# xianlopez/optical_flow

Measured on AMD Instinct MI355X. Metric: image-pairs/sec training, 384x512 batch=8 per GPU, higher is better.
Workload: dtype fp32

## Files before the change

### optical_flow_amd/csrc/conv_f32.hip

```cpp
#include "common.h"
#include "conv_dev.h"
#include "conv_narrow.h"

#include <algorithm>

namespace oflow {

template <int BM, int BN, int WAVES_M, int WAVES_N, int MODE>
__global__ __launch_bounds__(256, 2) void conv_gemm_f32(GemmArgs a) {
  constexpr int WM = BM / WAVES_M, WN = BN / WAVES_N;
  constexpr int TM = WM / 32, TN = WN / 32;
  static_assert(WAVES_M * WAVES_N == 4, "4 waves");
  static_assert(TM >= 1 && TN >= 1 && WM % 32 == 0 && WN % 32 == 0, "tile");
  constexpr bool A_KCONTIG = (MODE != MODE_WGRAD);
  constexpr int SA = BM + 4;
  constexpr int SB = BN + 4;
  constexpr int A_SLOTS = BM * BK / 4 / 256;
  constexpr int B_QUADS = BK * BN / 4;
  constexpr int B_SLOTS = (B_QUADS + 255) / 256;
  static_assert(A_SLOTS >= 1, "BM >= 64");

  static_assert(2 * BK * (SA + SB) >= 4 * 1024, "epilogue images fit LDS");
  __shared__ float smem[2 * BK * (SA + SB)];
  float (*As)[BK * SA] = reinterpret_cast<float (*)[BK * SA]>(smem);
// ... 602 lines not shown
      return;
    }
#pragma unroll
    for (int i = 0; i < TM; ++i)
#pragma unroll
      for (int j = 0; j < TN; ++j) {
        float4 vv[4];
        int64_t rows[4];
        unsigned ok = 0;
        int ncol = 0;
        transpose32(E, acc[i][j], lane, [&](int row, int c4, float4 v) {
          const int q = row >> 3;
          const int m = m0 + wm0 + 32 * i + row, n = n0 + wn0 + 32 * j + 4 * c4;
          if (a.splits > 1) {
            if (m < M && n < a.N)
              *reinterpret_cast<float4*>(&S[(int64_t)(row_base + m) * a.slab_ld + n]) = v;
            return;
          }
          rows[q] = out_row(a, G, min(m, M - 1));
          ok |= (m < M && n < a.N ? 1u : 0u) << q;
          vv[q] = v;
          ncol = n;
        });
        if (a.splits == 1) epilogue_rows4c<MODE, 4>(a, 0, rows, ok, ncol, min(ncol, a.N - 4), vv);
      }
    return;
  }
  if (a.splits > 1) {
    float* S = a.slab + (int64_t)split * a.split_stride;
    const int row_base = G.tiles_begin * BM;
#pragma unroll
    for (int j = 0; j < TN; ++j) {
      const int n = n0 + wn0 + 32 * j + lrow;
      if (n >= a.N) continue;
#pragma unroll
      for (int i = 0; i < TM; ++i)
#pragma unroll
        for (int r = 0; r < 16; ++r) {
          const int m = m0 + wm0 + 32 * i + (r & 3) + 8 * (r >> 2) + 4 * lk;
          if (m < M) S[(int64_t)(row_base + m) * a.slab_ld + n] = acc[i][j][r];
        }
    }
    return;
  }
#pragma unroll
  for (int j = 0; j < TN; ++j) {
    const int n = n0 + wn0 + 32 * j + lrow;
    if (n >= a.N) continue;
    float bias, scale, shift;
    column_params<MODE>(a, n, bias, scale, shift);
#pragma unroll
    for (int i = 0; i < TM; ++i) {
#pragma unroll
      for (int r0 = 0; r0 < 16; r0 += EP_GATHER<MODE>) {
        EpAux aux[EP_GATHER<MODE>];
#pragma unroll
        for (int r = r0; r < r0 + EP_GATHER<MODE>; ++r) {
          const int m = m0 + wm0 + 32 * i + (r & 3) + 8 * (r >> 2) + 4 * lk;
          aux[r - r0] = m < M ? epilogue_aux<MODE>(a, out_row(a, G, m), n) : EpAux{0.f, 0.f};
        }
#pragma unroll
        for (int r = r0; r < r0 + EP_GATHER<MODE>; ++r) {
          const int m = m0 + wm0 + 32 * i + (r & 3) + 8 * (r >> 2) + 4 * lk;
          if (m >= M) continue;
          epilogue_store<MODE>(a, out_row(a, G, m), n, acc[i][j][r], bias, scale, shift,
                               aux[r - r0]);
        }
      }
    }
  }
}

constexpr int TT_H = 8, TT_W = 16;
#ifndef OF_X3_TH0
#define OF_X3_TH0 8
#endif
constexpr int X3_TH0 = OF_X3_TH0;
#ifndef X3_ABL
#define X3_ABL 0
#endif
#ifndef X3_BDMA
#define X3_BDMA 1
#endif
#ifndef X3_EPB
#define X3_EPB 1
#endif

#ifndef X3_HREC
#define X3_HREC 1
#endif


template <int BN, int WAVES_M, int WAVES_N, int MODE, int TH = OF_TF_H, int PF = 1>
__global__ __launch_bounds__(64 * WAVES_M * WAVES_N, 256 / (32 * WAVES_M * WAVES_N)) void conv_tile_bf16(GemmArgs a) {
  constexpr bool g_tile16_pf_dev = PF != 0;
  constexpr int NT = 64 * WAVES_M * WAVES_N;
  constexpr int BM = TH * TF_W, KS = 3;
  constexpr int HH = TH + KS - 1, HW = TF_W + KS - 1, HP = HH * HW;
  constexpr int WM = BM / WAVES_M, WN = BN / WAVES_N;
  constexpr int TM = WM / 32, TN = WN / 32;
  static_assert((NT == 256 || NT == 512) && TM >= 1 && TN >= 1, "tile");
  constexpr int HQ = HP * 8, HS = (HQ + NT - 1) / NT;
  constexpr int BOCT = KS * BN * 4, BSL = (BOCT + NT - 1) / NT;
  static_assert((HP + 2 * KS * BN) * SROW16 * 16 >= (NT / 64) * 4096, "epilogue images fit LDS");
  __shared__ uint4 smem[(HP + 2 * KS * BN) * SROW16];
  uint4* Ah = smem;
  uint4 (*Bs)[KS * BN * SROW16] = reinterpret_cast<uint4 (*)[KS * BN * SROW16]>(smem + HP * SROW16);

  const int tid = threadIdx.x;
  const int lane = tid & 63;
  const int wave = __builtin_amdgcn_readfirstlane(tid >> 6);
  const int wgid = xcd_remap(blockIdx.x, gridDim.x);
  const int split = wgid / a.tiles_total;
  const int tile = wgid - split * a.tiles_total;
  const int tile_n = tile % a.n_tiles;
  const int tile_m = tile / a.n_tiles;
  const int n0 = tile_n * BN;
  const int OH = MODE == MODE_FWD ? a.ho : a.h, OW = MODE == MODE_FWD ? a.wo : a.w;
  const int SH = MODE == MODE_FWD ? a.h : a.ho, SW = MODE == MODE_FWD ? a.w : a.wo;
  const int tiles_x = (OW + TF_W - 1) / TF_W, tiles_y = (OH + TH - 1) / TH;
  const int b = tile_m / (tiles_x * tiles_y);
  const int trem = tile_m - b * tiles_x * tiles_y;
  const int oy0 = (trem / tiles_x) * TH, ox0 = (trem % tiles_x) * TF_W;
  const int hy0 = MODE == MODE_FWD ? oy0 - a.pt : oy0 + a.pt - (KS - 1);
  const int hx0 = MODE == MODE_FWD ? ox0 - a.pl : ox0 + a.pl - (KS - 1);
  const int c_begin = split * a.k_per_split;
  const int c_end = min(a.K, c_begin + a.k_per_split);
  const int steps = c_end > c_begin ? (c_end - c_begin) * KS : 0;

  const rsrc_t ra_src = make_rsrc(a.A, a.a_bytes);
  const rsrc_t rb_src = make_rsrc(a.B, a.b_bytes);

  int h_off[HS];
  unsigned h_ok = 0;
  const int hcq = tid & 7;
#pragma unroll
  for (int j = 0; j < HS; ++j) {
    const int q = tid + NT * j;
    const int hp = q >> 3;
    const int sy = hy0 + hp / HW, sx = hx0 + hp % HW;
    const bool ok = q < HQ && (unsigned)sy < (unsigned)SH && (unsigned)sx < (unsigned)SW;
    h_off[j] = ok ? (((b * SH + sy) * SW + sx) * a.lda + 4 * hcq) * 4 : 0;
    h_ok |= (ok ? 1u : 0u) << j;
  }
  float4 hv[HS];
  auto load_halo = [&](int c) {
    const bool cok = 32 * c + 4 * hcq < a.kc;
#pragma unroll
    for (int j = 0; j < HS; ++j)
      hv[j] = bload4(ra_src, cok && ((h_ok >> j) & 1) ? (uint32_t)(h_off[j] + 128 * c) : kOOB);
  };
  auto store_halo = [&]() {
#pragma unroll
    for (int j = 0; j < HS; ++j) {
      const int q = tid + NT * j;
      if (q < HQ) {
        bf16x8 t;
        const float4 v = hv[j];
        typedef __bf16 bf16x4 __attribute__((ext_vector_type(4)));
        bf16x4 u;
        u[0] = (__bf16)v.x;
        u[1] = (__bf16)v.y;
        u[2] = (__bf16)v.z;
        u[3] = (__bf16)v.w;
        (void)t;
        *reinterpret_cast<bf16x4*>(reinterpret_cast<char*>(Ah) + (q >> 3) * (SROW16 * 16) +
// ... 175 lines not shown
    __syncthreads();
    if (tid < BN / 4 && n0 + 4 * tid < a.N) {
      float4 sb = red[tid], sg = red[WAVES_M * (BN / 4) + tid];
      for (int w2 = 1; w2 < WAVES_M; ++w2) {
        add4(sb, red[w2 * (BN / 4) + tid]);
        add4(sg, red[(WAVES_M + w2) * (BN / 4) + tid]);
      }
      float* prow = a.bnp + (int64_t)tile_m * 2 * a.N + n0 + 4 * tid;
      *reinterpret_cast<float4*>(prow) = sb;
      *reinterpret_cast<float4*>(prow + a.N) = sg;
    }
    return;
  }
  if (a.vec_ep) {
    float* E = reinterpret_cast<float*>(smem) + wave * 1024;
#pragma unroll
    for (int i = 0; i < TM; ++i)
#pragma unroll
      for (int j = 0; j < TN; ++j) {
        float4 vv[4];
        int64_t rows[4];
        unsigned ok = 0;
        int ncol = 0;
        transpose32(E, acc[i][j], lane, [&](int row, int c4, float4 v) {
          const int q = row >> 3;
          const int mt = wm0 + 32 * i + row, n = n0 + wn0 + 32 * j + 4 * c4;
          const int oy = oy0 + mt / TF_W, ox = ox0 + mt % TF_W;
          rows[q] = img + (int64_t)min(oy, OH - 1) * OW + min(ox, OW - 1);
          ok |= (oy < OH && ox < OW && n < a.N ? 1u : 0u) << q;
          vv[q] = v;
          ncol = n;
        });
        epilogue_rows4c<MODE, 4>(a, split, rows, ok, ncol, min(ncol, a.N - 4), vv);
      }
    return;
  }
#pragma unroll
  for (int j = 0; j < TN; ++j) {
    const int n = n0 + wn0 + 32 * j + lrow;
    if (n >= a.N) continue;
    float bias = 0.f, scale = 1.f, shift = 0.f;
    if (a.splits == 1) column_params<MODE>(a, n, bias, scale, shift);
#pragma unroll
    for (int i = 0; i < TM; ++i) {
      EpAux aux[16];
#pragma unroll
      for (int rr = 0; rr < 16; ++rr) {
        const int m = wm0 + 32 * i + (rr & 3) + 8 * (rr >> 2) + 4 * lk;
        const int oy = oy0 + m / TF_W, ox = ox0 + m % TF_W;
        aux[rr] = a.splits == 1 && oy < OH && ox < OW
                      ? epilogue_aux<MODE>(a, img + (int64_t)oy * OW + ox, n) : EpAux{0.f, 0.f};
      }
#pragma unroll
      for (int rr = 0; rr < 16; ++rr) {
        const int m = wm0 + 32 * i + (rr & 3) + 8 * (rr >> 2) + 4 * lk;
        const int oy = oy0 + m / TF_W, ox = ox0 + m % TF_W;
        if (oy >= OH || ox >= OW) continue;
        const int64_t row = img + (int64_t)oy * OW + ox;
        if (a.splits > 1)
          a.slab[(int64_t)split * a.split_stride + row * a.slab_ld + n] = acc[i][j][rr];
        else
          epilogue_store<MODE>(a, row, n, acc[i][j][rr], bias, scale, shift, aux[rr]);
      }
    }
  }
}

__device__ __forceinline__ void split3x4(const float4& v, uint2& h, uint2& m, uint2& l) {
  const float x[4] = {v.x, v.y, v.z, v.w};
  uint32_t hb[4], mb[4], lb[4];
#pragma unroll
  for (int e = 0; e < 4; ++e) {
    hb[e] = __float_as_uint(x[e]) & 0xffff0000u;
    const float r = x[e] - __uint_as_float(hb[e]);
    mb[e] = __float_as_uint(r) & 0xffff0000u;
    lb[e] = __float_as_uint(r - __uint_as_float(mb[e]));
  }
  auto hi2 = [](uint32_t e0, uint32_t e1) { return __builtin_amdgcn_perm(e1, e0, 0x07060302u); };
  h = make_uint2(hi2(hb[0], hb[1]), hi2(hb[2], hb[3]));
  m = make_uint2(hi2(mb[0], mb[1]), hi2(mb[2], mb[3]));
  l = make_uint2(hi2(lb[0], lb[1]), hi2(lb[2], lb[3]));
}

template <int BN, int WAVES_M, int WAVES_N, int MODE, int TH, int NB, int NP>
__device__ __forceinline__ void tile_x3_body(const GemmArgs& a) {
  constexpr int BM = TH * TF_W, KS = 3;
  static_assert(NP == 1 || NP == 3, "planes");
  constexpr int HH = TH + KS - 1, HW = TF_W + KS - 1, HP = HH * HW;
  constexpr int WM = BM / WAVES_M, WN = BN / WAVES_N;
  constexpr int SM = WM / 16, SN = WN / 16;
  constexpr int NT = 64 * WAVES_M * WAVES_N;
  static_assert(NT % 64 == 0 && NT <= 1024 && WM % 16 == 0 && WN % 16 == 0 && SM >= 1 && SN >= 1,
                "tile");
  constexpr int HQ = HP * 8, HS = (HQ + NT - 1) / NT;
  constexpr int BOCT = NP * BN * 4, BSL = (BOCT + NT - 1) / NT;
  constexpr int AH_U4 = NP * HP * 4, BS_U4 = NB * NP * BN * 4;
  constexpr int EP1_U4 = (NT / 64) * WM * 16 * 4 / 16;
  constexpr int SM_U4 = AH_U4 + BS_U4 > EP1_U4 ? AH_U4 + BS_U4 : EP1_U4;
  constexpr int LDS_B = SM_U4 * 16;
  constexpr int EJ = (NT / 64) * WM * 16 * SN * 4 <= LDS_B ? SN
                     : (NT / 64) * WM * 8 * SN * 4 <= LDS_B ? SN / 2 : 1;
  constexpr int EPW = 16 * EJ;
  static_assert(SN % EJ == 0 && (NT / 64) * WM * EPW * 4 <= LDS_B, "epilogue image fits LDS");
  __shared__ uint4 smem[SM_U4];
  uint4* Ah = smem;
  uint4* Bs = smem + AH_U4;

  const int tid = threadIdx.x;
  const int lane = tid & 63;
  const int wave = __builtin_amdgcn_readfirstlane(tid >> 6);
  const int wgid = xcd_remap(blockIdx.x, gridDim.x);
  const int split = wgid / a.tiles_total;
  const int tile = wgid - split * a.tiles_total;
  const int tile_n = tile % a.n_tiles;
  const int tile_m = tile / a.n_tiles;
  const int n0 = tile_n * BN;
  const int OH = MODE == MODE_FWD ? a.ho : a.h, OW = MODE == MODE_FWD ? a.wo : a.w;
  const int SH = MODE == MODE_FWD ? a.h : a.ho, SW = MODE == MODE_FWD ? a.w : a.wo;
  const int tiles_x = (OW + TF_W - 1) / TF_W, tiles_y = (OH + TH - 1) / TH;
  const int b = tile_m / (tiles_x * tiles_y);
  const int trem = tile_m - b * tiles_x * tiles_y;
  const int oy0 = (trem / tiles_x) * TH, ox0 = (trem % tiles_x) * TF_W;
  const int hy0 = MODE == MODE_FWD ? oy0 - a.pt : oy0 + a.pt - (KS - 1);
  const int hx0 = MODE == MODE_FWD ? ox0 - a.pl : ox0 + a.pl - (KS - 1);
  const int c_begin = split * a.k_per_split;
  const int c_end = min(a.K, c_begin + a.k_per_split);

  const rsrc_t ra_src = make_rsrc(a.A, a.a_bytes);
  const rsrc_t rb_src = make_rsrc(a.B, a.b_bytes);

  float4 hv[HS];
  constexpr bool HREC = X3_HREC && NT == 256 && NP == 3;
  int h_off[HREC ? 1 : HS];
  unsigned h_ok = 0;
  const int hcq = tid & 7;
  auto halo_slot = [&](int t, int j, bool& ok) {
    const int q = t + NT * j;
    const int hp = q >> 3;
    const int sy = hy0 + hp / HW, sx = hx0 + hp % HW;
    ok = q < HQ && (unsigned)sy < (unsigned)SH && (unsigned)sx < (unsigned)SW;
    return ok ? (((b * SH + sy) * SW + sx) * a.lda + 4 * (t & 7)) * 4 : 0;
  };
  if constexpr (!HREC) {
#pragma unroll
    for (int j = 0; j < HS; ++j) {
      bool ok;
      h_off[j] = halo_slot(tid, j, ok);
      h_ok |= (ok ? 1u : 0u) << j;
    }
  }
  auto load_halo = [&](int c) {
    const bool cok = 32 * c + 4 * hcq < a.kc;
    if constexpr (HREC) {
      int t = tid;
      asm volatile("" : "+v"(t));
#pragma unroll
      for (int j = 0; j < HS; ++j) {
        bool ok;
        const int off = halo_slot(t, j, ok);
        hv[j] = bload4(ra_src, cok && ok ? (uint32_t)(off + 128 * c) : kOOB);
      }
    } else {
#pragma unroll
      for (int jj = 0; jj < HS; ++jj)
        hv[jj] = bload4(ra_src, cok && ((h_ok >> jj) & 1) ? (uint32_t)(h_off[jj] + 128 * c) : kOOB);
    }
  };
  auto store_halo = [&]() {
#pragma unroll
    for (int j = 0; j < HS; ++j) {
      const int q = tid + NT * j;
      if (q < HQ) {
        const int hp = q >> 3;
        const int off = hp * 64 + ((((q & 7) >> 1) ^ x3_sw(hp)) << 4) + 8 * (q & 1);
        char* base = reinterpret_cast<char*>(Ah);
        if constexpr (NP == 1) {
          *reinterpret_cast<uint2*>(base + off) = pack_bf16x4(hv[j]);
        } else {
          uint2 h, m, l;
          split3x4(hv[j], h, m, l);
          *reinterpret_cast<uint2*>(base + off) = h;
          *reinterpret_cast<uint2*>(base + HP * 64 + off) = m;
          *reinterpret_cast<uint2*>(base + 2 * HP * 64 + off) = l;
        }
      }
    }
  };
  uint32_t b_off[BSL];
  int b_lds[BSL];
#pragma unroll
  for (int j = 0; j < BSL; ++j) {
    const int o = tid + NT * j;
    const int p = o / (BN * 4), rem = o - p * (BN * 4);
    const int row = rem >> 2, oct = rem & 3;
    const int n = n0 + row;
    const bool ok = o < BOCT && n < a.nb;
    b_off[j] = ok ? (uint32_t)(((int64_t)p * a.b_plane + (int64_t)n * a.ldb + 8 * oct) * 2) : kOOB;
    b_lds[j] = o < BOCT ? (p * BN + row) * 4 + (oct ^ x3_sw(row)) : -1;
  }
  uint4 rb[BSL];
  auto load_b = [&](int c, int t) {
    const int so = (t * a.kc + 32 * c) * 2;
#pragma unroll
    for (int j = 0; j < BSL; ++j)
      rb[j] = __builtin_bit_cast(uint4, __builtin_amdgcn_raw_buffer_load_b128(rb_src, b_off[j], so, 0));
  };
  auto store_b = [&](int buf) {
#pragma unroll
    for (int j = 0; j < BSL; ++j)
      if (BOCT % NT == 0 || b_lds[j] >= 0) Bs[buf * NP * BN * 4 + b_lds[j]] = rb[j];
  };
  constexpr bool BDMA = X3_BDMA && NB == 2;
  constexpr int NW = NT / 64, BDI = NP * BN / 16, BDW = (BDI + NW - 1) / NW;
  uint32_t bd_off[BDW];
  int bd_lds[BDW];
#pragma unroll
  for (int k = 0; k < BDW; ++k) {
    const int g = wave + NW * k;
    const int p = g / (BN / 16), rbk = g % (BN / 16);
    const int n = rbk * 16 + (lane >> 2), o = (lane & 3) ^ x3_sw(lane >> 2);
    bd_off[k] = g < BDI && n0 + n < a.nb
                    ? (uint32_t)(((int64_t)p * a.b_plane + (int64_t)(n0 + n) * a.ldb + 8 * o) * 2)
                    : kOOB;
    bd_lds[k] = g < BDI ? (p * BN + rbk * 16) * 4 : -1;
  }
  auto dma_b = [&](int c, int t, int buf) {
    const int so = (t * a.kc + 32 * c) * 2;
#pragma unroll
    for (int k = 0; k < BDW; ++k)
      if (BDI % NW == 0 || bd_lds[k] >= 0)
        dma16_to_lds(rb_src, Bs + buf * NP * BN * 4 + bd_lds[k], bd_off[k], so);
  };

  f32x4 acc4[SM][SN];
#pragma unroll
  for (int i = 0; i < SM; ++i)
#pragma unroll
    for (int j = 0; j < SN; ++j)
#pragma unroll
      for (int r = 0; r < 4; ++r) acc4[i][j][r] = 0.f;
  const int wm0 = (wave / WAVES_N) * WM;
  const int wn0 = (wave % WAVES_N) * WN;
  const int l16 = lane & 15, lq = lane >> 4;
  int a_hp16[SM];
#pragma unroll
  for (int i = 0; i < SM; ++i) {
    const int m = wm0 + 16 * i + l16;
    const int ty = m / TF_W, tx = m % TF_W;
    a_hp16[i] = MODE == MODE_FWD ? ty * HW + tx : (ty + KS - 1) * HW + tx + KS - 1;
  }
  const int b_frag = (wn0 + l16) * 4 + (lq ^ x3_sw(l16));

  if (c_end > c_begin) {
    load_halo(c_begin);
    if constexpr (BDMA) dma_b(c_begin, 0, 0);
    else load_b(c_begin, 0);
    store_halo();
    if constexpr (!BDMA) store_b(0);
  }
  if constexpr (BDMA) asm volatile("s_waitcnt vmcnt(0)" ::: "memory");
  __syncthreads();
  for (int c = c_begin; c < c_end; ++c) {
    const int cc = c - c_begin;
    const bool more_c = c + 1 < c_end;
    if (more_c && !(X3_ABL & 4)) load_halo(c + 1);
#pragma unroll
    for (int t = 0; t < KS * KS; ++t) {
      const int buf = NB == 2 ? (cc + t) & 1 : 0;
      const bool more = t + 1 < KS * KS || more_c;
      if (more && !(X3_ABL & 2)) {
        if constexpr (BDMA) dma_b(t + 1 < KS * KS ? c : c + 1, t + 1 < KS * KS ? t + 1 : 0, buf ^ 1);
        else load_b(t + 1 < KS * KS ? c : c + 1, t + 1 < KS * KS ? t + 1 : 0);
      }
      __builtin_amdgcn_sched_barrier(0);
      const int r = t / KS, s = t % KS;
      const int dh = MODE == MODE_FWD ? r * HW + s : -(r * HW + s);
      bf16x8 av[NP][SM], bv[NP][SN];
#pragma unroll
      for (int i = 0; i < SM; ++i) {
        const int px = a_hp16[i] + dh;
        const int ai = px * 4 + (lq ^ x3_sw(px));
#pragma unroll
        for (int p = 0; p < NP; ++p) av[p][i] = __builtin_bit_cast(bf16x8, Ah[p * HP * 4 + ai]);
      }
#pragma unroll
      for (int p = 0; p < NP; ++p)
#pragma unroll
        for (int j = 0; j < SN; ++j)
          bv[p][j] = __builtin_bit_cast(bf16x8, Bs[(buf * NP + p) * BN * 4 + 64 * j + b_frag]);
#pragma unroll
      for (int i = 0; i < SM; ++i)
#pragma unroll
        for (int j = 0; j < SN; ++j) {
          f32x4 x = acc4[i][j];
          if constexpr (NP == 1) {
            acc4[i][j] = __builtin_amdgcn_mfma_f32_16x16x32_bf16(av[0][i], bv[0][j], x, 0, 0, 0);
            continue;
          } else {
          if (X3_ABL & 8) {
            asm volatile("" ::"v"(av[1][i]), "v"(av[2][i]), "v"(bv[1][j]), "v"(bv[2][j]));
            acc4[i][j] = __builtin_amdgcn_mfma_f32_16x16x32_bf16(av[0][i], bv[0][j], x, 0, 0, 0);
            continue;
          }
          x = __builtin_amdgcn_mfma_f32_16x16x32_bf16(av[2][i], bv[0][j], x, 0, 0, 0);
          x = __builtin_amdgcn_mfma_f32_16x16x32_bf16(av[0][i], bv[2][j], x, 0, 0, 0);
          x = __builtin_amdgcn_mfma_f32_16x16x32_bf16(av[1][i], bv[1][j], x, 0, 0, 0);
          x = __builtin_amdgcn_mfma_f32_16x16x32_bf16(av[1][i], bv[0][j], x, 0, 0, 0);
          x = __builtin_amdgcn_mfma_f32_16x16x32_bf16(av[0][i], bv[1][j], x, 0, 0, 0);
          acc4[i][j] = __builtin_amdgcn_mfma_f32_16x16x32_bf16(av[0][i], bv[0][j], x, 0, 0, 0);
          }
        }
      __builtin_amdgcn_sched_barrier(0);
      if (!(X3_ABL & 1) && (NB == 1 ? more : (t + 1 == KS * KS && more_c))) __syncthreads();
      if (more) {
        if (!(X3_ABL & 2) && !BDMA) store_b(NB == 2 ? buf ^ 1 : 0);
        if (t + 1 == KS * KS && more_c && !(X3_ABL & 4)) store_halo();
      }
      if constexpr (BDMA) asm volatile("s_waitcnt vmcnt(0)" ::: "memory");
      if (!(X3_ABL & 1)) __syncthreads();
    }
  }

  const int64_t img = (int64_t)b * OH * OW;
  if constexpr (X3_ABL & 16) {
    float v = 0.f;
#pragma unroll
    for (int i = 0; i < SM; ++i)
#pragma unroll
      for (int j = 0; j < SN; ++j) v += acc4[i][j][0] + acc4[i][j][1] + acc4[i][j][2] + acc4[i][j][3];
    a.C[(img + (int64_t)oy0 * OW + ox0) * a.ldc + (n0 + wn0 + (lane & 31)) % a.N] = v;
    return;
  }
  if constexpr (MODE == MODE_FWD && SM % 2 == 0 &&
                (NT / 64) * (WM / 2) * (WN * 4 + 32) <= LDS_B &&
                ((WM / 2) * (WN / 4)) % 64 == 0) {
    if (a.direct16) {
      direct_fwd_f32<SM, SN, WM, WN, TF_W>(
          a, acc4, reinterpret_cast<char*>(smem) + wave * (WM / 2) * (WN * 4 + 32), lane, wm0,
          wn0, n0, oy0, ox0, OH, OW, img);
      return;
    }
  }
  if constexpr (MODE == MODE_DGRAD && NT >= 512 && SM % 2 == 0 &&
                (NT / 64) * (WM / 2) * (WN * 4 + 32) <= LDS_B &&
                ((WM / 2) * (WN / 4)) % 64 == 0) {
    if (a.direct16) {
      direct_dgrad_f32<SM, SN, WM, WN, TF_W>(
          a, acc4, reinterpret_cast<char*>(smem) + wave * (WM / 2) * (WN * 4 + 32), lane, wm0,
          wn0, n0, oy0, ox0, OH, OW, img);
      return;
    }
  }
  if (a.vec_ep) {
    float* E = reinterpret_cast<float*>(smem) + wave * WM * EPW;
    constexpr int LPR = 4 * EJ, RPI = 64 / LPR;
    const int c4 = lane % LPR, rr = lane / LPR;
    constexpr int NPASS = SN / EJ;
    const bool bnp = MODE == MODE_DGRAD && a.bnp != nullptr;
    float4 bsb[NPASS], bsg[NPASS];
#pragma unroll
    for (int p = 0; p < NPASS; ++p) bsb[p] = bsg[p] = make_float4(0.f, 0.f, 0.f, 0.f);
#pragma unroll
    for (int jp = 0; jp < SN; jp += EJ) {
#pragma unroll
      for (int i = 0; i < SM; ++i)
#pragma unroll
        for (int j = 0; j < EJ; ++j)
#pragma unroll
          for (int r = 0; r < 4; ++r)
            E[(16 * i + 4 * lq + r) * EPW + 16 * j + l16] = acc4[i][jp + j][r];
      __builtin_amdgcn_fence(__ATOMIC_RELEASE, "wavefront");
      __builtin_amdgcn_wave_barrier();
      __builtin_amdgcn_fence(__ATOMIC_ACQUIRE, "wavefront");
      const int n = n0 + wn0 + 16 * jp + 4 * c4;
      if constexpr (X3_EPB > 1 && (WM / RPI) % X3_EPB == 0) {
#pragma unroll
        for (int q0 = 0; q0 < WM / RPI; q0 += X3_EPB) {
          float4 v[X3_EPB];
          int64_t row[X3_EPB];
          unsigned ok = 0;
#pragma unroll
          for (int g = 0; g < X3_EPB; ++g) {
            const int m = (q0 + g) * RPI + rr;
            v[g] = *reinterpret_cast<const float4*>(&E[m * EPW + 4 * c4]);
            const int mt = wm0 + m;
            const int oy = oy0 + mt / TF_W, ox = ox0 + mt % TF_W;
            row[g] = img + (int64_t)min(oy, OH - 1) * OW + min(ox, OW - 1);
            ok |= (oy < OH && ox < OW && n < a.N ? 1u : 0u) << g;
          }
          epilogue_rows4c<MODE, X3_EPB>(a, split, row, ok, n, min(n, a.N - 4), v);
        }
      } else if (MODE == MODE_DGRAD && bnp) {
        float4 bt = make_float4(0.f, 0.f, 0.f, 0.f), ig = bt;
        if (n < a.N) {
          bt = *reinterpret_cast<const float4*>(&a.bnp_b[n]);
          const float4 gm = *reinterpret_cast<const float4*>(&a.bnp_g[n]);
          ig = make_float4(1.f / gm.x, 1.f / gm.y, 1.f / gm.z, 1.f / gm.w);
        }
#pragma unroll
        for (int q = 0; q < WM / RPI; ++q) {
          const int m = q * RPI + rr;
          const float4 v = *reinterpret_cast<const float4*>(&E[m * EPW + 4 * c4]);
// ... 3012 lines not shown
  if (st || MODE == MODE_WGRAD || a.splits == 1) return st;
  return launch_splitk_epilogue<MODE>(a, s);
}

template <int MODE>
int launch_gemm_bf16(const GemmArgs& a, hipStream_t s, double flops) {
  const int bn = pick_bn(a.N);
  dim3 grid(a.tiles_total * a.splits), block(256);
  const int cfg = bn == 128 ? 0 : bn == 96 ? 1 : bn == 64 ? 2 : 3;
  if (timing_on()) timing_begin(s);
  if (cfg == 0) hipLaunchKernelGGL((conv_gemm_bf16<128, 128, 2, 2, MODE>), grid, block, 0, s, a);
  else if (cfg == 1) hipLaunchKernelGGL((conv_gemm_bf16<128, 96, 4, 1, MODE>), grid, block, 0, s, a);
  else if (cfg == 2) hipLaunchKernelGGL((conv_gemm_bf16<256, 64, 4, 1, MODE>), grid, block, 0, s, a);
  else hipLaunchKernelGGL((conv_gemm_bf16<256, 32, 4, 1, MODE>), grid, block, 0, s, a);
  if (timing_on()) timing_end(s, 64 + MODE * 8 + cfg, flops);
  int st = check_launch("conv_gemm_bf16");
  if (st || a.splits == 1) return st;
  return launch_splitk_epilogue<MODE>(a, s);
}

bool tile_ok(const of_conv_desc* d) { return d->kh == 3 && d->kw == 3 && d->stride == 1; }

bool x3_tall(int n, int oh, int ow, int N) {
  const int bn = pick_bn(N);
  return (bn == 128 || bn == 96) && (int64_t)n * cdiv(oh, X3_TH0) * cdiv(ow, TF_W) >= 4 * device_cus();
}

constexpr int X3_NB1_MIN = 384;
bool x3_nb1_candidate(const GemmArgs& a, bool tall) {
  return !tall && a.bn_tile == 0 && pick_bn(a.N) == 128 && a.tiles_total >= X3_NB1_MIN;
}
bool x3_nb1(const GemmArgs& a) {
  return a.bm != X3_TH0 * TF_W && a.splits == 1 && x3_nb1_candidate(a, false);
}

static int g_tile_b16 = 0;
bool ws_ok(const of_conv_desc* d, int mode) {
  const int N = mode == MODE_FWD ? d->cout : d->cin_p;
  return (g_tile_b16 == 2 || (g_tile_b16 == 3 && mode == MODE_FWD)) && pick_bn(N) >= 96;
}

static int g_x3t_ep = 5;
static int g_x3g_ep = 5;
static int g_x3_small_bn = 1200;
static int g_x3_bn64 = 0;
static int g_abl_noact = 0;
GemmArgs tile_args(const of_conv_desc* d, const Geo& g, int mode, bool x3 = false,
                   bool b16 = false, bool ws = false) {
  GemmArgs a = base_args(d);
  const bool fwd = mode == MODE_FWD;
  a.kc = fwd ? g.cin_p : g.cout_p;
  a.N = fwd ? d->cout : g.cin_p;
  a.nb = fwd ? d->cout : g.nd;
  a.ldb = fwd ? g.kf16 : (int)g.kd16;
  const int OH = fwd ? d->ho : d->h, OW = fwd ? d->wo : d->w;
  if (x3 && !b16 && !ws && g_x3_small_bn > 0 && pick_bn(a.N) == 128 &&
      (int64_t)d->n * cdiv(OH, TF_H) * cdiv(OW, TF_W) * cdiv(a.N, 128) < g_x3_small_bn)
    a.bn_tile = 64;
  const bool tall64 = x3 && !b16 && !ws && !a.bn_tile && g_x3_bn64 == 1 && pick_bn(a.N) == 64 &&
                      (int64_t)d->n * cdiv(OH, X3_TH0) * cdiv(OW, TF_W) >= 4 * device_cus();
  const bool tall = tall64 ? true : a.bn_tile ? false : ws ? true
                  : x3 || b16 ? x3_tall(d->n, OH, OW, a.N)
                             : (fwd || g_tall16_dgrad) && pick_bn(a.N) == 128 &&
                                   x3_tall(d->n, OH, OW, a.N);
  const int th = tall ? X3_TH0 : TF_H;
  const int m_tiles = d->n * (int)cdiv(OH, th) * (int)cdiv(OW, TF_W);
  a.bm = th * TF_W;
  a.ngroups = 1;
  Group& G = a.grp[0];
  G = Group{};
  G.M = d->n * OH * OW;
  G.m_tiles = m_tiles;
  G.ns = 3;
  G.ntaps = 9;
  a.M = G.M;
  a.n_tiles = (int)cdiv(a.N, a.bn_tile ? a.bn_tile : pick_bn(a.N));
  a.tiles_total = m_tiles * a.n_tiles;
  a.K = (int)cdiv(a.kc, 32);
  G.K = a.K;
  a.splits = 1;
  a.k_per_split = a.K;
  if (x3 || b16 || ws) {
    const bool bn64 = x3 && !b16 && !ws && (a.bn_tile ? a.bn_tile : pick_bn(a.N)) == 64;
    const int slots = !ws && ((b16 && !tall) || x3_nb1_candidate(a, tall) || a.bn_tile == 64 ||
                              (g_x3_bn64 && bn64))
                          ? 2 * device_cus() : device_cus();
    int best = 1;
    double best_cost = 1e30;
    for (int sp = 1; sp <= std::min(8, a.K); ++sp) {
      const int per = (int)cdiv(a.K, sp);
      if (cdiv(a.K, per) != sp) continue;
      const int64_t w = (int64_t)a.tiles_total * sp;
      const double cost = (double)cdiv(w, slots) * (per + 1.0) +
                          (sp > 1 ? 0.1 * g_x3t_ep * sp * a.tiles_total / (double)slots : 0.0);
      if (cost < best_cost - 1e-9) {
        best_cost = cost;
        best = sp;
      }
    }
    a.k_per_split = (int)cdiv(a.K, best);
    a.splits = (int)cdiv(a.K, a.k_per_split);
  } else if (a.tiles_total < 2 * device_cus()) {
    int sp = std::max(1, (4 * device_cus()) / a.tiles_total);
    sp = std::min(sp, std::max(1, a.K / 2));
    a.k_per_split = (int)cdiv(a.K, sp);
    a.splits = (int)cdiv(a.K, a.k_per_split);
  }
  return a;
}

template <int MODE>
int launch_tile_bf16(const GemmArgs& a, hipStream_t s, double flops) {
  const int bn = pick_bn(a.N);
  dim3 grid(a.tiles_total * a.splits), block(256);
  const bool tall = a.bm == X3_TH0 * TF_W;
  const int cfg = bn == 128 ? (tall ? 4 : 0) : bn == 96 ? 1 : bn == 64 ? 2 : 3;
  if (timing_on()) timing_begin(s);
  if (!g_tile16_pf) {
    if (cfg == 4) hipLaunchKernelGGL((conv_tile_bf16<128, 4, 2, MODE, X3_TH0, 0>), grid, dim3(512), 0, s, a);
    else if (cfg == 0) hipLaunchKernelGGL((conv_tile_bf16<128, 2, 2, MODE, OF_TF_H, 0>), grid, block, 0, s, a);
    else if (cfg == 1) hipLaunchKernelGGL((conv_tile_bf16<96, 4, 1, MODE, OF_TF_H, 0>), grid, block, 0, s, a);
    else if (cfg == 2) hipLaunchKernelGGL((conv_tile_bf16<64, 2, 2, MODE, OF_TF_H, 0>), grid, block, 0, s, a);
    else hipLaunchKernelGGL((conv_tile_bf16<32, 4, 1, MODE, OF_TF_H, 0>), grid, block, 0, s, a);
  } else if (cfg == 4) hipLaunchKernelGGL((conv_tile_bf16<128, 4, 2, MODE, X3_TH0>), grid, dim3(512), 0, s, a);
  else if (cfg == 0) hipLaunchKernelGGL((conv_tile_bf16<128, 2, 2, MODE>), grid, block, 0, s, a);
  else if (cfg == 1) hipLaunchKernelGGL((conv_tile_bf16<96, 4, 1, MODE>), grid, block, 0, s, a);
  else if (cfg == 2) hipLaunchKernelGGL((conv_tile_bf16<64, 2, 2, MODE>), grid, block, 0, s, a);
  else hipLaunchKernelGGL((conv_tile_bf16<32, 4, 1, MODE>), grid, block, 0, s, a);
  if (timing_on()) timing_end(s, 64 + 32 + MODE * 8 + cfg, flops);
  int st = check_launch("conv_tile_bf16");
  if (st || a.splits == 1) return st;
  return launch_splitk_epilogue<MODE>(a, s);
}

struct WgradPlan {
  int splits, k_per_split, M, ldc;
  int64_t split_stride;
};

template <int MODE>
int launch_tile_x3(const GemmArgs& a, hipStream_t s, double flops) {
  const int bn = a.bn_tile ? a.bn_tile : pick_bn(a.N);
  dim3 grid(a.tiles_total * a.splits), block(256);
  const bool tall = a.bm == X3_TH0 * TF_W;
  const int cfg = bn == 128 ? (tall ? 0 : x3_nb1(a) ? 4 : 6)
                            : bn == 96 ? (tall ? 5 : 1)
                            : bn == 64 ? (tall || g_x3_bn64 >= 2 ? 7 : 2) : 3;
  if (timing_on()) timing_begin(s);
  if (cfg == 7) {
    if (tall) hipLaunchKernelGGL((conv_tile_x3<64, 4, 1, MODE, X3_TH0, 1>), grid, block, 0, s, a);
    else if (g_x3_bn64 == 2) hipLaunchKernelGGL((conv_tile_x3<64, 4, 1, MODE, 4, 1>), grid, block, 0, s, a);
    else hipLaunchKernelGGL((conv_tile_x3<64, 2, 2, MODE, 4, 1>), grid, block, 0, s, a);
  } else if (cfg == 0) hipLaunchKernelGGL((conv_tile_x3<128, 4, 2, MODE, X3_TH0>), grid, dim3(512), 0, s, a);
  else if (cfg == 4) hipLaunchKernelGGL((conv_tile_x3<128, 2, 2, MODE, 4, 1>), grid, block, 0, s, a);
  else if (cfg == 6) hipLaunchKernelGGL((conv_tile_x3<128, 2, 4, MODE, 4>), grid, dim3(512), 0, s, a);
  else if (cfg == 5) hipLaunchKernelGGL((conv_tile_x3<96, 4, 3, MODE, X3_TH0>), grid, dim3(768), 0, s, a);
  else if (cfg == 1) hipLaunchKernelGGL((conv_tile_x3<96, 2, 3, MODE, 4>), grid, dim3(384), 0, s, a);
  else if (cfg == 2) hipLaunchKernelGGL((conv_tile_x3<64, 4, 2, MODE, 4>), grid, dim3(512), 0, s, a);
  else hipLaunchKernelGGL((conv_tile_x3<32, 4, 1, MODE, 4>), grid, block, 0, s, a);
  if (timing_on()) timing_end(s, 128 + MODE * 8 + cfg, flops);
  int st = check_launch("conv_tile_x3");
  if (st || a.splits == 1) return st;
  return launch_splitk_epilogue<MODE>(a, s);
}

template <int MODE>
int launch_tile_b16(const GemmArgs& a, hipStream_t s, double flops) {
// ... 1104 lines not shown
```

Measured before the change: 619.0.

## Add staged DMA ring pipeline for BN64 x3 conv tile with relaxed vmcnt waits

For the BN=64, 4x2-wave, TH=4, double-buffered three-plane bf16x3 conv tile, replaces the per-tap full vmcnt(0) wait plus double __syncthreads with a staged B-weight DMA scheme. The default mode is a 3-slot ring that prefetches two taps ahead. It waits with partial vmcnt counts, issues the next channel's halo loads early with precomputed addresses, and uses a single lgkmcnt+s_barrier per tap. The split-K slot heuristic is adjusted so the 2x-CU occupancy assumption depends on the stage mode. LDS use grows to three B slots, and correctness now relies on exact per-wave counting of outstanding vm ops.

After: 623.9 (median of 6 runs). No clear change (+0.8%).

```diff
diff --git a/optical_flow_amd/csrc/conv_f32.hip b/optical_flow_amd/csrc/conv_f32.hip
--- a/optical_flow_amd/csrc/conv_f32.hip
+++ b/optical_flow_amd/csrc/conv_f32.hip
@@ -708,6 +708,9 @@
 #ifndef X3_BDMA
 #define X3_BDMA 1
 #endif
+#ifndef X3_STG64
+#define X3_STG64 3
+#endif
 #ifndef X3_EPB
 #define X3_EPB 1
 #endif
@@ -1049,6 +1052,10 @@
   l = make_uint2(hi2(lb[0], lb[1]), hi2(lb[2], lb[3]));
 }
 
+constexpr int x3_stage(int bn, int waves_m, int waves_n, int th, int nb, int np) {
+  return X3_BDMA && np == 3 && bn == 64 && waves_m == 4 && waves_n == 2 && th == 4 && nb == 2
+             ? X3_STG64 : 0;
+}
 template <int BN, int WAVES_M, int WAVES_N, int MODE, int TH, int NB, int NP>
 __device__ __forceinline__ void tile_x3_body(const GemmArgs& a) {
   constexpr int BM = TH * TF_W, KS = 3;
@@ -1061,7 +1068,9 @@
                 "tile");
   constexpr int HQ = HP * 8, HS = (HQ + NT - 1) / NT;
   constexpr int BOCT = NP * BN * 4, BSL = (BOCT + NT - 1) / NT;
-  constexpr int AH_U4 = NP * HP * 4, BS_U4 = NB * NP * BN * 4;
+  constexpr int STG = x3_stage(BN, WAVES_M, WAVES_N, TH, NB, NP);
+  constexpr int NSLOT = STG == 2 ? 2 * KS : STG ? KS : NB;
+  constexpr int AH_U4 = NP * HP * 4, BS_U4 = NSLOT * NP * BN * 4;
   constexpr int EP1_U4 = (NT / 64) * WM * 16 * 4 / 16;
   constexpr int SM_U4 = AH_U4 + BS_U4 > EP1_U4 ? AH_U4 + BS_U4 : EP1_U4;
   constexpr int LDS_B = SM_U4 * 16;
@@ -1218,73 +1227,201 @@
   }
   const int b_frag = (wn0 + l16) * 4 + (lq ^ x3_sw(l16));
 
-  if (c_end > c_begin) {
-    load_halo(c_begin);
-    if constexpr (BDMA) dma_b(c_begin, 0, 0);
-    else load_b(c_begin, 0);
-    store_halo();
-    if constexpr (!BDMA) store_b(0);
-  }
-  if constexpr (BDMA) asm volatile("s_waitcnt vmcnt(0)" ::: "memory");
-  __syncthreads();
-  for (int c = c_begin; c < c_end; ++c) {
-    const int cc = c - c_begin;
-    const bool more_c = c + 1 < c_end;
-    if (more_c && !(X3_ABL & 4)) load_halo(c + 1);
-#pragma unroll
-    for (int t = 0; t < KS * KS; ++t) {
-      const int buf = NB == 2 ? (cc + t) & 1 : 0;
-      const bool more = t + 1 < KS * KS || more_c;
-      if (more && !(X3_ABL & 2)) {
-        if constexpr (BDMA) dma_b(t + 1 < KS * KS ? c : c + 1, t + 1 < KS * KS ? t + 1 : 0, buf ^ 1);
-        else load_b(t + 1 < KS * KS ? c : c + 1, t + 1 < KS * KS ? t + 1 : 0);
-      }
-      __builtin_amdgcn_sched_barrier(0);
-      const int r = t / KS, s = t % KS;
-      const int dh = MODE == MODE_FWD ? r * HW + s : -(r * HW + s);
-      bf16x8 av[NP][SM], bv[NP][SN];
-#pragma unroll
-      for (int i = 0; i < SM; ++i) {
-        const int px = a_hp16[i] + dh;
-        const int ai = px * 4 + (lq ^ x3_sw(px));
-#pragma unroll
-        for (int p = 0; p < NP; ++p) av[p][i] = __builtin_bit_cast(bf16x8, Ah[p * HP * 4 + ai]);
-      }
-#pragma unroll
-      for (int p = 0; p < NP; ++p)
-#pragma unroll
-        for (int j = 0; j < SN; ++j)
-          bv[p][j] = __builtin_bit_cast(bf16x8, Bs[(buf * NP + p) * BN * 4 + 64 * j + b_frag]);
-#pragma unroll
-      for (int i = 0; i < SM; ++i)
-#pragma unroll
-        for (int j = 0; j < SN; ++j) {
-          f32x4 x = acc4[i][j];
-          if constexpr (NP == 1) {
-            acc4[i][j] = __builtin_amdgcn_mfma_f32_16x16x32_bf16(av[0][i], bv[0][j], x, 0, 0, 0);
-            continue;
-          } else {
-          if (X3_ABL & 8) {
-            asm volatile("" ::"v"(av[1][i]), "v"(av[2][i]), "v"(bv[1][j]), "v"(bv[2][j]));
-            acc4[i][j] = __builtin_amdgcn_mfma_f32_16x16x32_bf16(av[0][i], bv[0][j], x, 0, 0, 0);
-            continue;
+  if constexpr (STG != 0) {
+    static_assert(BDMA && KS == 3 && HS + BDW <= 32, "x3 stage forms");
+    constexpr bool RING = STG == 3;
+    constexpr int TPS = RING ? 1 : KS;
+    const bool bd_full = wave + NW * (BDW - 1) < BDI;
+    auto lds_barrier = []() { asm volatile("s_waitcnt lgkmcnt(0)\n\ts_barrier" ::: "memory"); };
+    auto wait_but = [&](auto taps, auto extra) {
+      constexpr int T = decltype(taps)::value, E = decltype(extra)::value;
+      if (bd_full) asm volatile("s_waitcnt vmcnt(%0)" ::"n"(T * BDW + E) : "memory");
+      else asm volatile("s_waitcnt vmcnt(%0)" ::"n"(T * (BDW - 1) + E) : "memory");
+    };
+    using I0 = std::integral_constant<int, 0>;
+    using I1 = std::integral_constant<int, 1>;
+    using IH = std::integral_constant<int, HS>;
+    auto dma_stage = [&](int c, int t0, int slot0) {
+#pragma unroll
+      for (int u = 0; u < TPS; ++u) dma_b(c, t0 + u, slot0 + u);
+    };
+    static_assert(!HREC, "x3 stage forms keep h_off");
+    uint32_t h_nxt[HS];
+    auto halo_addr = [&](int c) {
+      const bool cok = 32 * c + 4 * hcq < a.kc;
+#pragma unroll
+      for (int jj = 0; jj < HS; ++jj) {
+        h_nxt[jj] = cok && ((h_ok >> jj) & 1) ? (uint32_t)(h_off[jj] + 128 * c) : kOOB;
+        asm volatile("" : "+v"(h_nxt[jj]));
+      }
+    };
+    auto load_halo_nxt = [&]() {
+#pragma unroll
+      for (int jj = 0; jj < HS; ++jj) hv[jj] = bload4(ra_src, h_nxt[jj]);
+    };
+    if (c_end > c_begin) {
+      load_halo(c_begin);
+      if constexpr (RING) dma_b(c_begin, 0, 0);
+      else dma_stage(c_begin, 0, 0);
+      store_halo();
+      if constexpr (RING) dma_b(c_begin, 1, 1);
+    }
+    halo_addr(c_begin + 1);
+    if constexpr (RING) wait_but(I1{}, I0{});
+    else wait_but(I0{}, I0{});
+    lds_barrier();
+    if (c_begin < c_end)
+      for (int c = c_begin;; ++c) {
+        const int cc = c - c_begin;
+        const bool more_c = c + 1 < c_end;
+#pragma unroll
+        for (int t = 0; t < KS * KS; ++t) {
+          const int r = t / KS, s = t % KS;
+          const int slot = STG == 2 ? ((cc + r) & 1) * KS + s : s;
+          const int dh = MODE == MODE_FWD ? r * HW + s : -(r * HW + s);
+          bf16x8 av[NP][SM], bv[NP][SN];
+#pragma unroll
+          for (int i = 0; i < SM; ++i) {
+            const int px = a_hp16[i] + dh;
+            const int ai = px * 4 + (lq ^ x3_sw(px));
+#pragma unroll
+            for (int p = 0; p < NP; ++p) av[p][i] = __builtin_bit_cast(bf16x8, Ah[p * HP * 4 + ai]);
           }
-          x = __builtin_amdgcn_mfma_f32_16x16x32_bf16(av[2][i], bv[0][j], x, 0, 0, 0);
-          x = __builtin_amdgcn_mfma_f32_16x16x32_bf16(av[0][i], bv[2][j], x, 0, 0, 0);
-          x = __builtin_amdgcn_mfma_f32_16x16x32_bf16(av[1][i], bv[1][j], x, 0, 0, 0);
-          x = __builtin_amdgcn_mfma_f32_16x16x32_bf16(av[1][i], bv[0][j], x, 0, 0, 0);
-          x = __builtin_amdgcn_mfma_f32_16x16x32_bf16(av[0][i], bv[1][j], x, 0, 0, 0);
-          acc4[i][j] = __builtin_amdgcn_mfma_f32_16x16x32_bf16(av[0][i], bv[0][j], x, 0, 0, 0);
+#pragma unroll
+          for (int p = 0; p < NP; ++p)
+#pragma unroll
+            for (int j = 0; j < SN; ++j)
+              bv[p][j] = __builtin_bit_cast(bf16x8, Bs[(slot * NP + p) * BN * 4 + 64 * j + b_frag]);
+          const bool issues = RING || (STG == 2 && s == 0);
+          if (issues) __builtin_amdgcn_sched_barrier(0);
+          if constexpr (RING) {
+            if (t + 2 < KS * KS) dma_b(c, t + 2, (t + 2) % KS);
+            else if (t + 2 == KS * KS && more_c) dma_b(c + 1, 0, 0);
+          } else if constexpr (STG == 2) {
+            if (s == 0) {
+              if (r + 1 < KS) dma_stage(c, t + KS, ((cc + r + 1) & 1) * KS);
+              else if (more_c) dma_stage(c + 1, 0, ((cc + r + 1) & 1) * KS);
+            }
+          }
+          if (t == 0 && more_c) {
+            asm volatile("" ::: "memory");
+            load_halo_nxt();
+          }
+          if (issues || t == 0) __builtin_amdgcn_sched_barrier(0);
+#pragma unroll
+          for (int i = 0; i < SM; ++i)
+#pragma unroll
+            for (int j = 0; j < SN; ++j) {
+              f32x4 x = acc4[i][j];
+              x = __builtin_amdgcn_mfma_f32_16x16x32_bf16(av[2][i], bv[0][j], x, 0, 0, 0);
+              x = __builtin_amdgcn_mfma_f32_16x16x32_bf16(av[0][i], bv[2][j], x, 0, 0, 0);
+              x = __builtin_amdgcn_mfma_f32_16x16x32_bf16(av[1][i], bv[1][j], x, 0, 0, 0);
+              x = __builtin_amdgcn_mfma_f32_16x16x32_bf16(av[1][i], bv[0][j], x, 0, 0, 0);
+              x = __builtin_amdgcn_mfma_f32_16x16x32_bf16(av[0][i], bv[1][j], x, 0, 0, 0);
+              acc4[i][j] = __builtin_amdgcn_mfma_f32_16x16x32_bf16(av[0][i], bv[0][j], x, 0, 0, 0);
+            }
+          if (RING || s == KS - 1) __builtin_amdgcn_sched_barrier(0);
+          const bool last = t + 1 == KS * KS;
+          if (last) continue;
+          if constexpr (RING) {
+            if (t + 2 == KS * KS) {
+              if (more_c) wait_but(I1{}, I0{});
+              else wait_but(I0{}, I0{});
+            } else if (t < 2 && more_c) {
+              wait_but(I1{}, IH{});
+            } else {
+              wait_but(I1{}, I0{});
+            }
+            lds_barrier();
+          } else if (s == KS - 1) {
+            if constexpr (STG == 1) {
+              lds_barrier();
+              dma_stage(c, t + 1, 0);
+            }
+            wait_but(I0{}, I0{});
+            lds_barrier();
           }
         }
-      __builtin_amdgcn_sched_barrier(0);
-      if (!(X3_ABL & 1) && (NB == 1 ? more : (t + 1 == KS * KS && more_c))) __syncthreads();
-      if (more) {
-        if (!(X3_ABL & 2) && !BDMA) store_b(NB == 2 ? buf ^ 1 : 0);
-        if (t + 1 == KS * KS && more_c && !(X3_ABL & 4)) store_halo();
-      }
-      if constexpr (BDMA) asm volatile("s_waitcnt vmcnt(0)" ::: "memory");
-      if (!(X3_ABL & 1)) __syncthreads();
+        if (!more_c) break;
+        lds_barrier();
+        if constexpr (STG == 1) dma_stage(c + 1, 0, 0);
+        store_halo();
+        if constexpr (RING) dma_b(c + 1, 1, 1);
+        halo_addr(c + 2);
+        if constexpr (RING) wait_but(I1{}, I0{});
+        else wait_but(I0{}, I0{});
+        lds_barrier();
+      }
+    lds_barrier();
+  } else {
+    if (c_end > c_begin) {
+      load_halo(c_begin);
+      if constexpr (BDMA) dma_b(c_begin, 0, 0);
+      else load_b(c_begin, 0);
+      store_halo();
+      if constexpr (!BDMA) store_b(0);
+    }
+    if constexpr (BDMA) asm volatile("s_waitcnt vmcnt(0)" ::: "memory");
+    __syncthreads();
+    for (int c = c_begin; c < c_end; ++c) {
+      const int cc = c - c_begin;
+      const bool more_c = c + 1 < c_end;
+      if (more_c && !(X3_ABL & 4)) load_halo(c + 1);
+#pragma unroll
+      for (int t = 0; t < KS * KS; ++t) {
+        const int buf = NB == 2 ? (cc + t) & 1 : 0;
+        const bool more = t + 1 < KS * KS || more_c;
+        if (more && !(X3_ABL & 2)) {
+          if constexpr (BDMA) dma_b(t + 1 < KS * KS ? c : c + 1, t + 1 < KS * KS ? t + 1 : 0, buf ^ 1);
+          else load_b(t + 1 < KS * KS ? c : c + 1, t + 1 < KS * KS ? t + 1 : 0);
+        }
+        __builtin_amdgcn_sched_barrier(0);
+        const int r = t / KS, s = t % KS;
+        const int dh = MODE == MODE_FWD ? r * HW + s : -(r * HW + s);
+        bf16x8 av[NP][SM], bv[NP][SN];
+#pragma unroll
+        for (int i = 0; i < SM; ++i) {
+          const int px = a_hp16[i] + dh;
+          const int ai = px * 4 + (lq ^ x3_sw(px));
+#pragma unroll
+          for (int p = 0; p < NP; ++p) av[p][i] = __builtin_bit_cast(bf16x8, Ah[p * HP * 4 + ai]);
+        }
+#pragma unroll
+        for (int p = 0; p < NP; ++p)
+#pragma unroll
+          for (int j = 0; j < SN; ++j)
+            bv[p][j] = __builtin_bit_cast(bf16x8, Bs[(buf * NP + p) * BN * 4 + 64 * j + b_frag]);
+#pragma unroll
+        for (int i = 0; i < SM; ++i)
+#pragma unroll
+          for (int j = 0; j < SN; ++j) {
+            f32x4 x = acc4[i][j];
+            if constexpr (NP == 1) {
+              acc4[i][j] = __builtin_amdgcn_mfma_f32_16x16x32_bf16(av[0][i], bv[0][j], x, 0, 0, 0);
+              continue;
+            } else {
+            if (X3_ABL & 8) {
+              asm volatile("" ::"v"(av[1][i]), "v"(av[2][i]), "v"(bv[1][j]), "v"(bv[2][j]));
+              acc4[i][j] = __builtin_amdgcn_mfma_f32_16x16x32_bf16(av[0][i], bv[0][j], x, 0, 0, 0);
+              continue;
+            }
+            x = __builtin_amdgcn_mfma_f32_16x16x32_bf16(av[2][i], bv[0][j], x, 0, 0, 0);
+            x = __builtin_amdgcn_mfma_f32_16x16x32_bf16(av[0][i], bv[2][j], x, 0, 0, 0);
+            x = __builtin_amdgcn_mfma_f32_16x16x32_bf16(av[1][i], bv[1][j], x, 0, 0, 0);
+            x = __builtin_amdgcn_mfma_f32_16x16x32_bf16(av[1][i], bv[0][j], x, 0, 0, 0);
+            x = __builtin_amdgcn_mfma_f32_16x16x32_bf16(av[0][i], bv[1][j], x, 0, 0, 0);
+            acc4[i][j] = __builtin_amdgcn_mfma_f32_16x16x32_bf16(av[0][i], bv[0][j], x, 0, 0, 0);
+            }
+          }
+        __builtin_amdgcn_sched_barrier(0);
+        if (!(X3_ABL & 1) && (NB == 1 ? more : (t + 1 == KS * KS && more_c))) __syncthreads();
+        if (more) {
+          if (!(X3_ABL & 2) && !BDMA) store_b(NB == 2 ? buf ^ 1 : 0);
+          if (t + 1 == KS * KS && more_c && !(X3_ABL & 4)) store_halo();
+        }
+        if constexpr (BDMA) asm volatile("s_waitcnt vmcnt(0)" ::: "memory");
+        if (!(X3_ABL & 1)) __syncthreads();
+      }
     }
   }
 
@@ -4463,7 +4600,8 @@
   a.k_per_split = a.K;
   if (x3 || b16 || ws) {
     const bool bn64 = x3 && !b16 && !ws && (a.bn_tile ? a.bn_tile : pick_bn(a.N)) == 64;
-    const int slots = !ws && ((b16 && !tall) || x3_nb1_candidate(a, tall) || a.bn_tile == 64 ||
+    const bool bn64_two = a.bn_tile == 64 && (g_x3_bn64 >= 2 || x3_stage(64, 4, 2, 4, 2, 3) != 2);
+    const int slots = !ws && ((b16 && !tall) || x3_nb1_candidate(a, tall) || bn64_two ||
                               (g_x3_bn64 && bn64))
                           ? 2 * device_cus() : device_cus();
     int best = 1;
```
